# LiqunZhao/Neural-ordinary-differential-equations-based-Lyapunov-Barrier-Actor-Critic-NLBAC

Hardware: AMD Instinct MI355X
Metric: ODE-integrate+update samples/sec, Unicycle batch 4096 (higher is better)
Workload: dtype f32; 1 GPU; Unicycle B=4096 dopri5 (BASELINE.json configs[1] at B=4096 dopri5); NODE fit on 32768 rows every 10 updates; replay of 65536 synthetic transitions resident in HBM; solver=dopri5, adjoint=False, batch_per_gpu=4096, global_batch=4096, node_fit_rows_per_gpu=32768, parallelism=dp1, hipgraph=False

## Files before the change

neural-ordinary-differential-equations-based-lyapunov-barrier-actor-critic-nlbac_amd/csrc/mlp_dw16_kernels.hip:

```cpp
#include "common.h"
#include "mlp_launch.h"
#include "rr_device.h"

typedef float f32x2 __attribute__((ext_vector_type(2)));
#define DW16_PF 8
#define DW16_OOB ((int)0x80000000)

__device__ __forceinline__ int dw16_col(int t, int i) { return t < 4 ? 4 * i + t : (t < 6 ? 64 + 2 * i + (t - 4) : 96 + i); }

template <int NT, bool VEC>
struct Dw16Side {
    static constexpr int T = VEC ? NT : 1;
    __amdgpu_buffer_rsrc_t rs;
    int vo4, vo2, vo1;
    const float* p0; const float* p1;
    int ld0, ld1, split, width, nrows, q, i;
    float v[DW16_PF][T];

    __device__ __forceinline__ void init_vec(const float* base, int hid, int B, int q_, int i_) {
        rs = rr_rsrc(base, B * hid);
        q = q_; i = i_; width = hid; nrows = B;
        const int row = q * hid * 4;
        vo4 = (4 * i + 3 < hid) ? row + 16 * i : DW16_OOB;
        vo2 = (64 + 2 * i + 1 < hid) ? row + 256 + 8 * i : DW16_OOB;
        vo1 = (96 + i < hid) ? row + 384 + 4 * i : DW16_OOB;
    }
    __device__ __forceinline__ void init_gather(const float* a, int lda, int split_, const float* b, int ldb, int width_,
                                                int B, int q_, int i_) {
        p0 = a; p1 = b; ld0 = lda; ld1 = ldb; split = split_; width = width_; nrows = B; q = q_; i = i_;
    }
    __device__ __forceinline__ void load(int u, int g) {
        if constexpr (VEC) {
            const int rb = g * 16 * width;
            const f32x4 a = rr_ldw(rs, vo4 + rb, 0);
            v[u][0] = a[0]; v[u][1] = a[1]; v[u][2] = a[2]; v[u][3] = a[3];
            if constexpr (NT > 4) {
                const f32x2 b = __builtin_bit_cast(f32x2, __builtin_amdgcn_raw_buffer_load_b64(rs, vo2 + rb, 0, 0));
                v[u][4] = b[0];
                v[u][5] = b[1];
            }
            if constexpr (NT > 6) v[u][6] = __builtin_bit_cast(float, __builtin_amdgcn_raw_buffer_load_b32(rs, vo1 + rb, 0, 0));
        } else {
            const long row = 4L * g + q;
            float x = 0.f;
            if (i < width && row < nrows) x = (i < split) ? p0[row * ld0 + i] : p1[row * ld1 + (i - split)];
            v[u][0] = x;
        }
    }
};

template <int NT, bool AVEC, bool BVEC>
__device__ __forceinline__ void dw16_body(Dw16Side<NT, AVEC>& a, Dw16Side<NT, BVEC>& b, int g0, int gstep, int n_ksteps,
                                          float* __restrict__ gW, int ldw, float* __restrict__ gb, float* smem) {
    constexpr int NTA = Dw16Side<NT, AVEC>::T, NTB = Dw16Side<NT, BVEC>::T;
    const int tid = threadIdx.x, lane = tid & 63, wave = tid >> 6, q = lane >> 4, i = lane & 15;
    f32x4 acc[NTA][NTB];
    float bs[NTA];
#pragma unroll
    for (int ta = 0; ta < NTA; ++ta) {
        bs[ta] = 0.f;
#pragma unroll
        for (int tb = 0; tb < NTB; ++tb) acc[ta][tb] = f32x4{0.f, 0.f, 0.f, 0.f};
    }
    const int mine = (g0 < n_ksteps) ? (n_ksteps - g0 + gstep - 1) / gstep : 0;
    const int rounds = (mine + DW16_PF - 1) / DW16_PF;
    if (rounds > 0) {
#pragma unroll
        for (int u = 0; u < DW16_PF; ++u) { a.load(u, g0 + u * gstep); b.load(u, g0 + u * gstep); }
        int g = g0 + DW16_PF * gstep;
        for (int r = 0; r < rounds; ++r) {
#pragma unroll
            for (int u = 0; u < DW16_PF; ++u) {
                float av[NTA], bv[NTB];
#pragma unroll
                for (int t = 0; t < NTA; ++t) { av[t] = a.v[u][t]; bs[t] += av[t]; }
#pragma unroll
                for (int t = 0; t < NTB; ++t) bv[t] = b.v[u][t];
#ifndef DW16_NO_MFMA
#pragma unroll
                for (int ta = 0; ta < NTA; ++ta)
#pragma unroll
                    for (int tb = 0; tb < NTB; ++tb)
                        acc[ta][tb] = __builtin_amdgcn_mfma_f32_16x16x4f32(av[ta], bv[tb], acc[ta][tb], 0, 0, 0);
#endif
#pragma unroll
                for (int ta = 0; ta < NTA; ++ta)
#pragma unroll
                    for (int tb = 0; tb < NTB; ++tb) asm volatile("" : "+a"(acc[ta][tb]));
#ifndef DW16_NO_LOAD
                a.load(u, g);
                b.load(u, g);
#endif
                __builtin_amdgcn_sched_barrier(0);
                g += gstep;
            }
        }
    }

    float* red = smem;
    for (int w = 1; w < 4; ++w) {
        __syncthreads();
        if (wave == w) {
#pragma unroll
            for (int ta = 0; ta < NTA; ++ta)
#pragma unroll
                for (int tb = 0; tb < NTB; ++tb)
#pragma unroll
                    for (int r = 0; r < 4; ++r) red[((ta * NTB + tb) * 4 + r) * 64 + lane] = acc[ta][tb][r];
        }
        __syncthreads();
        if (wave == 0) {
#pragma unroll
            for (int ta = 0; ta < NTA; ++ta)
#pragma unroll
                for (int tb = 0; tb < NTB; ++tb)
#pragma unroll
                    for (int r = 0; r < 4; ++r) acc[ta][tb][r] += red[((ta * NTB + tb) * 4 + r) * 64 + lane];
        }
    }
    __syncthreads();
    float (*sBias)[NTA * 16] = reinterpret_cast<float (*)[NTA * 16]>(smem);
#pragma unroll
    for (int t = 0; t < NTA; ++t) sBias[wave * 4 + q][t * 16 + i] = bs[t];
    __syncthreads();
    if (tid < NTA * 16) {
        float v = 0.f;
#pragma unroll
        for (int k = 0; k < 16; ++k) v += sBias[k][tid];
        const int col = AVEC ? dw16_col(tid >> 4, tid & 15) : (tid & 15);
        if (col < a.width) gb[col] = v;
    }
    if (wave == 0) {
#pragma unroll
        for (int ta = 0; ta < NTA; ++ta)
#pragma unroll
            for (int tb = 0; tb < NTB; ++tb)
#pragma unroll
                for (int r = 0; r < 4; ++r) {
                    const int n = AVEC ? dw16_col(ta, 4 * q + r) : 4 * q + r;
                    const int k = BVEC ? dw16_col(tb, i) : i;
                    if (n < a.width && k < b.width) gW[(long)n * ldw + k] = acc[ta][tb][r];
                }
    }
}

__device__ __forceinline__ int dw16_layer_of_slot(int slot, int nwide) {
    return slot < nwide - 1 ? slot + 1 : (slot == nwide - 1 ? 0 : nwide);
}

template <int NT>
__global__ __launch_bounds__(256) void mlp_dw16_kernel(const MlpLaunch L) {
    extern __shared__ __attribute__((aligned(16))) float dw16_smem[];
    const nlbac_mlp& net = L.net[blockIdx.y];
    const nlbac_mlp_io& io = L.io[blockIdx.y];
    const int B = L.B, hid = net.hid, nwide = net.n_layers - 1;
    if ((int)blockIdx.z > nwide) return;
    const int j = dw16_layer_of_slot(blockIdx.z, nwide);
#ifdef DW16_NO_EDGE
    if (j == 0 || j == nwide) return;
#endif
#ifdef DW16_NO_WIDE
    if (j != 0 && j != nwide) return;
#endif
    const int slab = blockIdx.x;
    const int lane = threadIdx.x & 63, wave = threadIdx.x >> 6, q = lane >> 4, i = lane & 15;
    const int g0 = slab * 4 + wave, gstep = L.n_slabs * 4, n_ksteps = (B + 3) >> 2;
    const long ls = io.acts_ls ? io.acts_ls : (long)B * hid;
    float* g = io.grad + (long)slab * L.slab_stride;
    if (j == 0) {
        Dw16Side<NT, true> a; Dw16Side<NT, false> b;
        a.init_vec(io.dz, hid, B, q, i);
        b.init_gather(io.x0, io.x0_ld, io.x0_dim, io.x1, io.x1_ld, net.in_dim, B, q, i);
        dw16_body<NT, true, false>(a, b, g0, gstep, n_ksteps, g + net.w_off[0], net.in_dim, g + net.b_off[0], dw16_smem);
    } else if (j == nwide) {
        Dw16Side<NT, false> a; Dw16Side<NT, true> b;
        a.init_gather(io.dy, io.dy_ld, net.out_dim, nullptr, 0, net.out_dim, B, q, i);
        b.init_vec(io.acts + (long)(nwide - 1) * ls, hid, B, q, i);
        dw16_body<NT, false, true>(a, b, g0, gstep, n_ksteps, g + net.w_off[nwide], hid, g + net.b_off[nwide], dw16_smem);
    } else {
        Dw16Side<NT, true> a; Dw16Side<NT, true> b;
        a.init_vec(io.dz + (long)j * ls, hid, B, q, i);
        b.init_vec(io.acts + (long)(j - 1) * ls, hid, B, q, i);
        dw16_body<NT, true, true>(a, b, g0, gstep, n_ksteps, g + net.w_off[j], hid, g + net.b_off[j], dw16_smem);
    }
}

bool nlbac_mlp_dw16_eligible(const nlbac_mlp* nets, int n_nets, int B) {
    static const bool on = [] { const char* e = getenv("NLBAC_MLP_DW16"); return !(e && e[0] == '0'); }();
    if (!on) return false;
    for (int i = 0; i < n_nets; ++i)
        if (nets[i].hid > 112) return false;
    return true;
}

int nlbac_mlp_dw16_launch(const MlpLaunch& L, int n_nets, hipStream_t s) {
    int max_hid = 0, max_layers = 0;
    for (int i = 0; i < n_nets; ++i) {
        NLBAC_REQUIRE(((long)L.B + 16L * DW16_PF * L.n_slabs + 4) * L.net[i].hid < (1L << 29),
                      "nlbac_mlp_bwd_weights: %d rows x %d units (+ the ring's run-out) exceed 2^29 elements per layer", L.B, L.net[i].hid);
        if (L.net[i].hid > max_hid) max_hid = L.net[i].hid;
        if (L.net[i].n_layers > max_layers) max_layers = L.net[i].n_layers;
    }
    const dim3 grid(L.n_slabs, n_nets, max_layers);
    const size_t lds = (size_t)49 * 4 * 64 * sizeof(float);
    if (max_hid <= 64) hipLaunchKernelGGL(mlp_dw16_kernel<4>, grid, dim3(256), lds, s, L);
    else if (max_hid <= 96) hipLaunchKernelGGL(mlp_dw16_kernel<6>, grid, dim3(256), lds, s, L);
    else hipLaunchKernelGGL(mlp_dw16_kernel<7>, grid, dim3(256), lds, s, L);
    NLBAC_CHECK_LAUNCH("nlbac_mlp_bwd_weights(dw16)");
    return 0;
}
```

Measured before the change: 3.649 million samples/s.

## Fold edge-layer weight-gradient jobs into wide-layer blocks of dw16 kernel

Adds a FOLD variant of the dw16 weight-gradient kernel. When the grid would exceed the CU count, the small first and last layer jobs are co-scheduled inside wide-layer blocks and share one load/MFMA loop, using a shallower prefetch ring to limit register pressure. This removes the separate thin blocks for edge layers, which underuse MFMA, at the cost of more per-block work and a reduced prefetch depth. It also simplifies the gather loads to a single precomputed pointer with a clamped row instead of a branch.

```diff
diff --git a/neural-ordinary-differential-equations-based-lyapunov-barrier-actor-critic-nlbac_amd/csrc/mlp_dw16_kernels.hip b/neural-ordinary-differential-equations-based-lyapunov-barrier-actor-critic-nlbac_amd/csrc/mlp_dw16_kernels.hip
--- a/neural-ordinary-differential-equations-based-lyapunov-barrier-actor-critic-nlbac_amd/csrc/mlp_dw16_kernels.hip
+++ b/neural-ordinary-differential-equations-based-lyapunov-barrier-actor-critic-nlbac_amd/csrc/mlp_dw16_kernels.hip
@@ -4,18 +4,19 @@
 
 typedef float f32x2 __attribute__((ext_vector_type(2)));
 #define DW16_PF 8
+#define DW16_PF_FOLD 4
 #define DW16_OOB ((int)0x80000000)
 
 __device__ __forceinline__ int dw16_col(int t, int i) { return t < 4 ? 4 * i + t : (t < 6 ? 64 + 2 * i + (t - 4) : 96 + i); }
 
-template <int NT, bool VEC>
+template <int NT, bool VEC, int RD = DW16_PF>
 struct Dw16Side {
     static constexpr int T = VEC ? NT : 1;
     __amdgpu_buffer_rsrc_t rs;
     int vo4, vo2, vo1;
-    const float* p0; const float* p1;
-    int ld0, ld1, split, width, nrows, q, i;
-    float v[DW16_PF][T];
+    const float* p0;
+    int ld0, width, nrows, q, i;
+    float v[RD][T];
 
     __device__ __forceinline__ void init_vec(const float* base, int hid, int B, int q_, int i_) {
         rs = rr_rsrc(base, B * hid);
@@ -25,9 +26,12 @@
         vo2 = (64 + 2 * i + 1 < hid) ? row + 256 + 8 * i : DW16_OOB;
         vo1 = (96 + i < hid) ? row + 384 + 4 * i : DW16_OOB;
     }
-    __device__ __forceinline__ void init_gather(const float* a, int lda, int split_, const float* b, int ldb, int width_,
+    __device__ __forceinline__ void init_gather(const float* a, int lda, int split, const float* b, int ldb, int width_,
                                                 int B, int q_, int i_) {
-        p0 = a; p1 = b; ld0 = lda; ld1 = ldb; split = split_; width = width_; nrows = B; q = q_; i = i_;
+        width = width_; nrows = B; q = q_; i = i_;
+        const bool first = i < split || i >= width;
+        p0 = first ? a + (i < split ? i : 0) : b + (i - split);
+        ld0 = first ? lda : ldb;
     }
     __device__ __forceinline__ void load(int u, int g) {
         if constexpr (VEC) {
@@ -41,114 +45,154 @@
             }
             if constexpr (NT > 6) v[u][6] = __builtin_bit_cast(float, __builtin_amdgcn_raw_buffer_load_b32(rs, vo1 + rb, 0, 0));
         } else {
-            const long row = 4L * g + q;
-            float x = 0.f;
-            if (i < width && row < nrows) x = (i < split) ? p0[row * ld0 + i] : p1[row * ld1 + (i - split)];
-            v[u][0] = x;
+            const int row = 4 * g + q;
+            const bool ok = i < width && row < nrows;
+            const float x = p0[(long)(ok ? row : 0) * ld0];
+            v[u][0] = ok ? x : 0.f;
         }
     }
 };
 
-template <int NT, bool AVEC, bool BVEC>
-__device__ __forceinline__ void dw16_body(Dw16Side<NT, AVEC>& a, Dw16Side<NT, BVEC>& b, int g0, int gstep, int n_ksteps,
-                                          float* __restrict__ gW, int ldw, float* __restrict__ gb, float* smem) {
-    constexpr int NTA = Dw16Side<NT, AVEC>::T, NTB = Dw16Side<NT, BVEC>::T;
-    const int tid = threadIdx.x, lane = tid & 63, wave = tid >> 6, q = lane >> 4, i = lane & 15;
+template <int NT, bool AVEC, bool BVEC, int RD = DW16_PF>
+struct Dw16Prod {
+    static constexpr int NTA = Dw16Side<NT, AVEC>::T, NTB = Dw16Side<NT, BVEC>::T;
+    Dw16Side<NT, AVEC, RD> a;
+    Dw16Side<NT, BVEC, RD> b;
     f32x4 acc[NTA][NTB];
     float bs[NTA];
-#pragma unroll
-    for (int ta = 0; ta < NTA; ++ta) {
-        bs[ta] = 0.f;
-#pragma unroll
-        for (int tb = 0; tb < NTB; ++tb) acc[ta][tb] = f32x4{0.f, 0.f, 0.f, 0.f};
-    }
+
+    __device__ __forceinline__ void zero() {
+#pragma unroll
+        for (int ta = 0; ta < NTA; ++ta) {
+            bs[ta] = 0.f;
+#pragma unroll
+            for (int tb = 0; tb < NTB; ++tb) acc[ta][tb] = f32x4{0.f, 0.f, 0.f, 0.f};
+        }
+    }
+    __device__ __forceinline__ void load(int u, int g) { a.load(u, g); b.load(u, g); }
+    __device__ __forceinline__ void step(int u) {
+        float av[NTA], bv[NTB];
+#pragma unroll
+        for (int t = 0; t < NTA; ++t) { av[t] = a.v[u][t]; bs[t] += av[t]; }
+#pragma unroll
+        for (int t = 0; t < NTB; ++t) bv[t] = b.v[u][t];
+#ifndef DW16_NO_MFMA
+#pragma unroll
+        for (int ta = 0; ta < NTA; ++ta)
+#pragma unroll
+            for (int tb = 0; tb < NTB; ++tb)
+                acc[ta][tb] = __builtin_amdgcn_mfma_f32_16x16x4f32(av[ta], bv[tb], acc[ta][tb], 0, 0, 0);
+#endif
+    }
+    __device__ __forceinline__ void anchor() {
+#pragma unroll
+        for (int ta = 0; ta < NTA; ++ta)
+#pragma unroll
+            for (int tb = 0; tb < NTB; ++tb) asm volatile("" : "+a"(acc[ta][tb]));
+    }
+    __device__ __forceinline__ void finish(float* __restrict__ gW, int ldw, float* __restrict__ gb, float* smem) {
+        const int tid = threadIdx.x, lane = tid & 63, wave = tid >> 6, q = lane >> 4, i = lane & 15;
+        float* red = smem;
+        for (int w = 1; w < 4; ++w) {
+            __syncthreads();
+            if (wave == w) {
+#pragma unroll
+                for (int ta = 0; ta < NTA; ++ta)
+#pragma unroll
+                    for (int tb = 0; tb < NTB; ++tb)
+#pragma unroll
+                        for (int r = 0; r < 4; ++r) red[((ta * NTB + tb) * 4 + r) * 64 + lane] = acc[ta][tb][r];
+            }
+            __syncthreads();
+            if (wave == 0) {
+#pragma unroll
+                for (int ta = 0; ta < NTA; ++ta)
+#pragma unroll
+                    for (int tb = 0; tb < NTB; ++tb)
+#pragma unroll
+                        for (int r = 0; r < 4; ++r) acc[ta][tb][r] += red[((ta * NTB + tb) * 4 + r) * 64 + lane];
+            }
+        }
+        __syncthreads();
+        float (*sBias)[NTA * 16] = reinterpret_cast<float (*)[NTA * 16]>(smem);
+#pragma unroll
+        for (int t = 0; t < NTA; ++t) sBias[wave * 4 + q][t * 16 + i] = bs[t];
+        __syncthreads();
+        if (tid < NTA * 16) {
+            float v = 0.f;
+#pragma unroll
+            for (int k = 0; k < 16; ++k) v += sBias[k][tid];
+            const int col = AVEC ? dw16_col(tid >> 4, tid & 15) : (tid & 15);
+            if (col < a.width) gb[col] = v;
+        }
+        if (wave == 0) {
+#pragma unroll
+            for (int ta = 0; ta < NTA; ++ta)
+#pragma unroll
+                for (int tb = 0; tb < NTB; ++tb)
+#pragma unroll
+                    for (int r = 0; r < 4; ++r) {
+                        const int n = AVEC ? dw16_col(ta, 4 * q + r) : 4 * q + r;
+                        const int k = BVEC ? dw16_col(tb, i) : i;
+                        if (n < a.width && k < b.width) gW[(long)n * ldw + k] = acc[ta][tb][r];
+                    }
+        }
+    }
+};
+
+struct Dw16None {
+    __device__ __forceinline__ void zero() {}
+    __device__ __forceinline__ void load(int, int) {}
+    __device__ __forceinline__ void step(int) {}
+    __device__ __forceinline__ void anchor() {}
+};
+
+template <int RD, class P, class Q>
+__device__ __forceinline__ void dw16_run(P& p, Q& e, int g0, int gstep, int n_ksteps) {
+    static_assert(DW16_PF % RD == 0, "the ring depth divides DW16_PF");
+    p.zero(); e.zero();
     const int mine = (g0 < n_ksteps) ? (n_ksteps - g0 + gstep - 1) / gstep : 0;
-    const int rounds = (mine + DW16_PF - 1) / DW16_PF;
+    const int rounds = (mine + DW16_PF - 1) / DW16_PF * (DW16_PF / RD);
     if (rounds > 0) {
 #pragma unroll
-        for (int u = 0; u < DW16_PF; ++u) { a.load(u, g0 + u * gstep); b.load(u, g0 + u * gstep); }
-        int g = g0 + DW16_PF * gstep;
+        for (int u = 0; u < RD; ++u) { p.load(u, g0 + u * gstep); e.load(u, g0 + u * gstep); }
+        int g = g0 + RD * gstep;
         for (int r = 0; r < rounds; ++r) {
 #pragma unroll
-            for (int u = 0; u < DW16_PF; ++u) {
-                float av[NTA], bv[NTB];
-#pragma unroll
-                for (int t = 0; t < NTA; ++t) { av[t] = a.v[u][t]; bs[t] += av[t]; }
-#pragma unroll
-                for (int t = 0; t < NTB; ++t) bv[t] = b.v[u][t];
-#ifndef DW16_NO_MFMA
-#pragma unroll
-                for (int ta = 0; ta < NTA; ++ta)
-#pragma unroll
-                    for (int tb = 0; tb < NTB; ++tb)
-                        acc[ta][tb] = __builtin_amdgcn_mfma_f32_16x16x4f32(av[ta], bv[tb], acc[ta][tb], 0, 0, 0);
-#endif
-#pragma unroll
-                for (int ta = 0; ta < NTA; ++ta)
-#pragma unroll
-                    for (int tb = 0; tb < NTB; ++tb) asm volatile("" : "+a"(acc[ta][tb]));
+            for (int u = 0; u < RD; ++u) {
+                p.step(u);
+                e.step(u);
+                if constexpr (RD == DW16_PF) { p.anchor(); e.anchor(); }
 #ifndef DW16_NO_LOAD
-                a.load(u, g);
-                b.load(u, g);
+                p.load(u, g);
+                e.load(u, g);
 #endif
                 __builtin_amdgcn_sched_barrier(0);
                 g += gstep;
             }
         }
     }
-
-    float* red = smem;
-    for (int w = 1; w < 4; ++w) {
-        __syncthreads();
-        if (wave == w) {
-#pragma unroll
-            for (int ta = 0; ta < NTA; ++ta)
-#pragma unroll
-                for (int tb = 0; tb < NTB; ++tb)
-#pragma unroll
-                    for (int r = 0; r < 4; ++r) red[((ta * NTB + tb) * 4 + r) * 64 + lane] = acc[ta][tb][r];
-        }
-        __syncthreads();
-        if (wave == 0) {
-#pragma unroll
-            for (int ta = 0; ta < NTA; ++ta)
-#pragma unroll
-                for (int tb = 0; tb < NTB; ++tb)
-#pragma unroll
-                    for (int r = 0; r < 4; ++r) acc[ta][tb][r] += red[((ta * NTB + tb) * 4 + r) * 64 + lane];
-        }
-    }
-    __syncthreads();
-    float (*sBias)[NTA * 16] = reinterpret_cast<float (*)[NTA * 16]>(smem);
-#pragma unroll
-    for (int t = 0; t < NTA; ++t) sBias[wave * 4 + q][t * 16 + i] = bs[t];
-    __syncthreads();
-    if (tid < NTA * 16) {
-        float v = 0.f;
-#pragma unroll
-        for (int k = 0; k < 16; ++k) v += sBias[k][tid];
-        const int col = AVEC ? dw16_col(tid >> 4, tid & 15) : (tid & 15);
-        if (col < a.width) gb[col] = v;
-    }
-    if (wave == 0) {
-#pragma unroll
-        for (int ta = 0; ta < NTA; ++ta)
-#pragma unroll
-            for (int tb = 0; tb < NTB; ++tb)
-#pragma unroll
-                for (int r = 0; r < 4; ++r) {
-                    const int n = AVEC ? dw16_col(ta, 4 * q + r) : 4 * q + r;
-                    const int k = BVEC ? dw16_col(tb, i) : i;
-                    if (n < a.width && k < b.width) gW[(long)n * ldw + k] = acc[ta][tb][r];
-                }
-    }
 }
 
 __device__ __forceinline__ int dw16_layer_of_slot(int slot, int nwide) {
     return slot < nwide - 1 ? slot + 1 : (slot == nwide - 1 ? 0 : nwide);
 }
 
-template <int NT>
+template <int NT, int RD>
+__device__ __forceinline__ void dw16_init_first(Dw16Prod<NT, true, false, RD>& p, const nlbac_mlp& net, const nlbac_mlp_io& io,
+                                                int B, int q, int i) {
+    p.a.init_vec(io.dz, net.hid, B, q, i);
+    p.b.init_gather(io.x0, io.x0_ld, io.x0_dim, io.x1, io.x1_ld, net.in_dim, B, q, i);
+}
+template <int NT, int RD>
+__device__ __forceinline__ void dw16_init_last(Dw16Prod<NT, false, true, RD>& p, const nlbac_mlp& net, const nlbac_mlp_io& io,
+                                               int B, long ls, int q, int i) {
+    const int nwide = net.n_layers - 1;
+    p.a.init_gather(io.dy, io.dy_ld, net.out_dim, nullptr, 0, net.out_dim, B, q, i);
+    p.b.init_vec(io.acts + (long)(nwide - 1) * ls, net.hid, B, q, i);
+}
+
+template <int NT, bool FOLD>
 __global__ __launch_bounds__(256) void mlp_dw16_kernel(const MlpLaunch L) {
     extern __shared__ __attribute__((aligned(16))) float dw16_smem[];
     const nlbac_mlp& net = L.net[blockIdx.y];
@@ -156,32 +200,63 @@
     const int B = L.B, hid = net.hid, nwide = net.n_layers - 1;
     if ((int)blockIdx.z > nwide) return;
     const int j = dw16_layer_of_slot(blockIdx.z, nwide);
+    const bool edge = j == 0 || j == nwide;
 #ifdef DW16_NO_EDGE
-    if (j == 0 || j == nwide) return;
+    if (edge) return;
 #endif
 #ifdef DW16_NO_WIDE
-    if (j != 0 && j != nwide) return;
-#endif
+    if (!edge) return;
+#endif
+    int ejob = -1;
+    if constexpr (FOLD) {
+        if (edge) return;
+        int widx = blockIdx.z;
+        for (int n = 0; n < (int)blockIdx.y; ++n) widx += L.net[n].n_layers - 2;
+        if (widx < 2 * (int)gridDim.y) ejob = widx;
+    }
     const int slab = blockIdx.x;
     const int lane = threadIdx.x & 63, wave = threadIdx.x >> 6, q = lane >> 4, i = lane & 15;
     const int g0 = slab * 4 + wave, gstep = L.n_slabs * 4, n_ksteps = (B + 3) >> 2;
     const long ls = io.acts_ls ? io.acts_ls : (long)B * hid;
     float* g = io.grad + (long)slab * L.slab_stride;
-    if (j == 0) {
-        Dw16Side<NT, true> a; Dw16Side<NT, false> b;
-        a.init_vec(io.dz, hid, B, q, i);
-        b.init_gather(io.x0, io.x0_ld, io.x0_dim, io.x1, io.x1_ld, net.in_dim, B, q, i);
-        dw16_body<NT, true, false>(a, b, g0, gstep, n_ksteps, g + net.w_off[0], net.in_dim, g + net.b_off[0], dw16_smem);
-    } else if (j == nwide) {
-        Dw16Side<NT, false> a; Dw16Side<NT, true> b;
-        a.init_gather(io.dy, io.dy_ld, net.out_dim, nullptr, 0, net.out_dim, B, q, i);
-        b.init_vec(io.acts + (long)(nwide - 1) * ls, hid, B, q, i);
-        dw16_body<NT, false, true>(a, b, g0, gstep, n_ksteps, g + net.w_off[nwide], hid, g + net.b_off[nwide], dw16_smem);
+    if (!FOLD && j == 0) {
+        Dw16Prod<NT, true, false> p; Dw16None none;
+        dw16_init_first(p, net, io, B, q, i);
+        dw16_run<DW16_PF>(p, none, g0, gstep, n_ksteps);
+        p.finish(g + net.w_off[0], net.in_dim, g + net.b_off[0], dw16_smem);
+    } else if (!FOLD && j == nwide) {
+        Dw16Prod<NT, false, true> p; Dw16None none;
+        dw16_init_last(p, net, io, B, ls, q, i);
+        dw16_run<DW16_PF>(p, none, g0, gstep, n_ksteps);
+        p.finish(g + net.w_off[nwide], hid, g + net.b_off[nwide], dw16_smem);
     } else {
-        Dw16Side<NT, true> a; Dw16Side<NT, true> b;
-        a.init_vec(io.dz + (long)j * ls, hid, B, q, i);
-        b.init_vec(io.acts + (long)(j - 1) * ls, hid, B, q, i);
-        dw16_body<NT, true, true>(a, b, g0, gstep, n_ksteps, g + net.w_off[j], hid, g + net.b_off[j], dw16_smem);
+        constexpr int RD = FOLD ? DW16_PF_FOLD : DW16_PF;
+        Dw16Prod<NT, true, true, RD> p;
+        p.a.init_vec(io.dz + (long)j * ls, hid, B, q, i);
+        p.b.init_vec(io.acts + (long)(j - 1) * ls, hid, B, q, i);
+        if (ejob < 0) {
+            Dw16None none;
+            dw16_run<RD>(p, none, g0, gstep, n_ksteps);
+            p.finish(g + net.w_off[j], hid, g + net.b_off[j], dw16_smem);
+            return;
+        }
+        const nlbac_mlp& en = L.net[ejob >> 1];
+        const nlbac_mlp_io& eio = L.io[ejob >> 1];
+        float* eg = eio.grad + (long)slab * L.slab_stride;
+        if ((ejob & 1) == 0) {
+            Dw16Prod<NT, true, false, RD> e;
+            dw16_init_first(e, en, eio, B, q, i);
+            dw16_run<RD>(p, e, g0, gstep, n_ksteps);
+            p.finish(g + net.w_off[j], hid, g + net.b_off[j], dw16_smem);
+            e.finish(eg + en.w_off[0], en.in_dim, eg + en.b_off[0], dw16_smem);
+        } else {
+            const int enw = en.n_layers - 1;
+            Dw16Prod<NT, false, true, RD> e;
+            dw16_init_last(e, en, eio, B, eio.acts_ls ? eio.acts_ls : (long)B * en.hid, q, i);
+            dw16_run<RD>(p, e, g0, gstep, n_ksteps);
+            p.finish(g + net.w_off[j], hid, g + net.b_off[j], dw16_smem);
+            e.finish(eg + en.w_off[enw], en.hid, eg + en.b_off[enw], dw16_smem);
+        }
     }
 }
 
@@ -194,18 +269,27 @@
 }
 
 int nlbac_mlp_dw16_launch(const MlpLaunch& L, int n_nets, hipStream_t s) {
-    int max_hid = 0, max_layers = 0;
+    int max_hid = 0, max_layers = 0, n_wide = 0;
     for (int i = 0; i < n_nets; ++i) {
         NLBAC_REQUIRE(((long)L.B + 16L * DW16_PF * L.n_slabs + 4) * L.net[i].hid < (1L << 29),
                       "nlbac_mlp_bwd_weights: %d rows x %d units (+ the ring's run-out) exceed 2^29 elements per layer", L.B, L.net[i].hid);
         if (L.net[i].hid > max_hid) max_hid = L.net[i].hid;
         if (L.net[i].n_layers > max_layers) max_layers = L.net[i].n_layers;
-    }
+        n_wide += L.net[i].n_layers - 2;
+    }
+    static const int n_cus = [] {
+        int dev = 0, n = 0;
+        if (hipGetDevice(&dev) != hipSuccess || hipDeviceGetAttribute(&n, hipDeviceAttributeMultiprocessorCount, dev) != hipSuccess) n = 0;
+        return n;
+    }();
+    const bool fold = n_wide >= 2 * n_nets && (long)(n_wide + 2 * n_nets) * L.n_slabs > n_cus;
     const dim3 grid(L.n_slabs, n_nets, max_layers);
     const size_t lds = (size_t)49 * 4 * 64 * sizeof(float);
-    if (max_hid <= 64) hipLaunchKernelGGL(mlp_dw16_kernel<4>, grid, dim3(256), lds, s, L);
-    else if (max_hid <= 96) hipLaunchKernelGGL(mlp_dw16_kernel<6>, grid, dim3(256), lds, s, L);
-    else hipLaunchKernelGGL(mlp_dw16_kernel<7>, grid, dim3(256), lds, s, L);
+    void (*k)(const MlpLaunch) = nullptr;
+    if (max_hid <= 64) k = fold ? mlp_dw16_kernel<4, true> : mlp_dw16_kernel<4, false>;
+    else if (max_hid <= 96) k = fold ? mlp_dw16_kernel<6, true> : mlp_dw16_kernel<6, false>;
+    else k = fold ? mlp_dw16_kernel<7, true> : mlp_dw16_kernel<7, false>;
+    hipLaunchKernelGGL(k, grid, dim3(256), lds, s, L);
     NLBAC_CHECK_LAUNCH("nlbac_mlp_bwd_weights(dw16)");
     return 0;
 }
```

New measurement: 3.360 million samples/s. 7.9% lower.
